# geobacter-rs/rav1e

Hardware: AMD Instinct MI355X
Metric: encoded frames/sec + Mpixels/sec, 4K 8-bit speed=10, 1/2/4/8 GPU vs host CPU (higher is better)
Workload: dtype u8

## Files before the change

rav1e_amd/csrc/rv_rdo.h:

```cpp
#pragma once

#include "rv_chain.h"
#include "rv_device.h"
#include "rv_quant.h"

namespace rv {

struct RdoPlane {
  rv_plane org;
  rv_plane ref[2];
  rv_plane dst;
  int32_t *levels;
  uint64_t *out;
  QCtx q;
};

struct RdoWinner {
  int32_t c;
  int32_t skip;
  double cost;
  uint64_t dist;
};

struct RdoArgs {
  RdoPlane p[2];
  CandGeo g;
  const rv_fs_result *sub;
  const RdoWinner *win;
  const float *imp;
  int w_in_b, h_in_b, w_imp;
  int n_tx;
  int cand_base;
  const int32_t *list;
  const int32_t *count;
  int commit;
  int ntx_per_cand;
  int bd;
  int bsize;
  int mb_w, mb_h;
  int sub_w, sub_h;
  int xdec, ydec;
  int q_tx_index;
  int tx_size, qindex;
  const void *iedges;
  const uint8_t *imodes;
  const uint8_t *iwin;
};

}

int rv_quant_ctx(int qindex, int tx_area, int is_intra, int bit_depth, int dc_delta_q,
                 int ac_delta_q, rv::QCtx *out);

int rv_rdo_candidates(const rv::RdoArgs &luma, const rv::RdoArgs &chroma, int hbd,
                      hipStream_t s, bool compound = false);

int rv_rdo_blocks2(const rv::RdoArgs &l, const rv::RdoArgs &c, int nl, int nc, int hbd,
                   hipStream_t s, int mode);
int rv_rdo_blocks(const rv::RdoArgs &a, bool luma, int nplanes, int n_tx_size, int hbd,
                  hipStream_t s, int mode);

int rv_rdo_args_put(const rv::RdoArgs *h, int n, rv::RdoArgs *dev, hipStream_t s);
int rv_rdo_candidates_list(const rv::RdoArgs *h, const rv::RdoArgs *dev, int nsets, int mode_a,
                           int hbd, hipStream_t s, int max_grid = 0, uint32_t *kp_cnt = nullptr,
                           unsigned long long *kp_t = nullptr);

int rv_rdo_intra(const rv::RdoArgs &luma, const rv::RdoArgs &chroma, int hbd, hipStream_t s);
```

rav1e_amd/csrc/rv_rdo.hip:

```cpp
#include <stdio.h>
#include <stdlib.h>
#include <string.h>

#include <type_traits>

#include "rv_intra.h"
#include "rv_rdo.h"
#include "rv_tx.h"

namespace rv {


__constant__ int8_t kRdoReg[2][16][8] = {
    {{0, 0, 0, 127, 0, 0, 0, 0}, {0, 2, -6, 126, 8, -2, 0, 0},
     {0, 2, -10, 122, 18, -4, 0, 0}, {0, 2, -12, 116, 28, -8, 2, 0},
     {0, 2, -14, 110, 38, -10, 2, 0}, {0, 2, -14, 102, 48, -12, 2, 0},
     {0, 2, -16, 94, 58, -12, 2, 0}, {0, 2, -14, 84, 66, -12, 2, 0},
     {0, 2, -14, 76, 76, -14, 2, 0}, {0, 2, -12, 66, 84, -14, 2, 0},
     {0, 2, -12, 58, 94, -16, 2, 0}, {0, 2, -12, 48, 102, -14, 2, 0},
     {0, 2, -10, 38, 110, -14, 2, 0}, {0, 2, -8, 28, 116, -12, 2, 0},
     {0, 0, -4, 18, 122, -10, 2, 0}, {0, 0, -2, 8, 126, -6, 2, 0}},
    {{0, 0, 0, 127, 0, 0, 0, 0}, {0, 0, -4, 126, 8, -2, 0, 0},
     {0, 0, -8, 122, 18, -4, 0, 0}, {0, 0, -10, 116, 28, -6, 0, 0},
     {0, 0, -12, 110, 38, -8, 0, 0}, {0, 0, -12, 102, 48, -10, 0, 0},
// ... 81 lines not shown
  wave_sync();
  IntraSetup st = intra_setup(jb.imode, jb.ivar);
  if (st.mode == 0) st.dcv = intra_dc<G>(e, jb.ivar, N, N, bd, lane);
  const int maxv = (1 << bd) - 1;
  for (int i = lane; i < N * N; i += G) {
    const int r = i / N, c = i - r * N;
    pred[i] = (Px)intra_px(st, e, N, N, r, c, maxv);
  }
  wave_sync();
}

__device__ __forceinline__ int rdo_ntx(const RdoArgs &a) {
  return a.count ? __builtin_amdgcn_readfirstlane(*a.count) * a.ntx_per_cand : a.n_tx;
}

template <int N>
__device__ __forceinline__ RdoJob rdo_job(const RdoArgs &a, const RdoPlane &pl, int t) {
  const int ci = t / a.ntx_per_cand, sub = t - ci * a.ntx_per_cand;
  const int cand = a.list ? a.list[ci] : a.cand_base + ci;
  int sb, c;
  RdoJob j;
  j.zero = false;
  j.oi = cand * a.ntx_per_cand + sub;
  if (a.commit) {
    sb = cand;
    c = a.win[sb].c;
    j.zero = a.win[sb].skip != 0;
  } else {
    c = cand / a.g.nsb;
    sb = cand - c * a.g.nsb;
  }
  rv_mv mv, mv1{0, 0};
  j.comp = c >= a.g.R * a.g.M;
  if (j.comp) {
// ... 11 lines not shown
  j.oy = (sub / txc) * N;
  const rv_mc_job m = mc_job_for(pl.ref[j.ref], j.bx, j.by, mv, 0, 0);
  j.src_x = m.src_x;
  j.src_y = m.src_y;
  j.cf = m.col_frac;
  j.rf = m.row_frac;
  j.src2_x = j.src2_y = j.cf2 = j.rf2 = 0;
  if (j.comp) {
    const rv_mc_job m1 = mc_job_for(pl.ref[1], j.bx, j.by, mv1, 0, 0);
    j.src2_x = m1.src_x;
    j.src2_y = m1.src_y;
    j.cf2 = m1.col_frac;
    j.rf2 = m1.row_frac;
  }
  return j;
}

struct McF {
  uint32_t xp[3];
  int xsum;
  int yt[8];
  int cf, rf;
};
template <typename Px>
__device__ __forceinline__ McF mc_setup(int cf, int rf, int w, int h) {
  McF f;
  f.cf = cf;
  f.rf = rf;
  const int8_t *xf = kRdoReg[w <= 4][cf];
  const int8_t *yf = kRdoReg[h <= 4][rf];
// ... 220 lines not shown
  }
}

template <typename Px, int N>
__host__ __device__ constexpr int rdo_slab_bytes() {
  constexpr int B = (int)sizeof(Px);
  constexpr int P = B == 1 ? ((N + 8 + 15) / 16) * 16 : ((2 * (N + 8) + 15) / 16) * 16;
  constexpr int RB = N < 16 ? N : 16;
  constexpr int a = N * (N + 1) * 4, b = (N + 7) * P, c = 2 * (RB + 7) * P;
  return ((a > b ? a : b) > c ? (a > b ? a : b) : c);
}

template <typename Px, int N, int LPB, int MODE, bool LUMA = false>
__device__ __forceinline__ void rdo_cand_body(const RdoArgs &a, const RdoPlane &pl, int t,
                                              bool valid, int32_t *buf, Px *pred,
                                              const uint16_t *scan) {
  constexpr int B = (int)sizeof(Px);
  constexpr int S = N + 1;
  constexpr int G = LPB / N, RG = N / G;
  constexpr int U = RG < 8 ? RG : 8;
  constexpr int P = B == 1 ? ((N + 8 + 15) / 16) * 16 : ((2 * (N + 8) + 15) / 16) * 16;
  constexpr int C32 = N < 32 ? N : 32;
  static_assert(!LUMA || N >= 8, "cdef distortion runs on 8x8 blocks");
  const int lane = rv_tid() & (LPB - 1);
  RdoJob jb;
  if constexpr (MODE == 3)
    jb = rdo_job_intra<Px, N>(a, &pl == &a.p[1] ? 2 : 1, t);
  else
    jb = rdo_job<N>(a, pl, t);
  const rv_plane &ref = pl.ref[jb.ref];
  const int ox = jb.ox, oy = jb.oy;
  const int bd = a.bd, ib = bd == 12 ? 2 : 4, maxv = (1 << bd) - 1;
  const int sx0 = jb.bx + ox, sy0 = jb.by + oy;
  auto wave_sync = [] {
    __builtin_amdgcn_fence(__ATOMIC_RELEASE, "wavefront");
    __builtin_amdgcn_wave_barrier();
    __builtin_amdgcn_fence(__ATOMIC_ACQUIRE, "wavefront");
  };

  if constexpr (MODE == 3) {
    intra_fill<Px, N, LPB>(jb, buf, pred, a.bd, lane);
  } else if (MODE == 1 || (MODE == 2 && jb.comp)) {
    static_assert(2 * (16 + 7) * (sizeof(Px) == 1 ? 48 : 80) <= N * (N + 1) * 4 || N != 32,
                  "compound windows must fit the coefficient slab");
// ... 205 lines not shown
#pragma unroll 8
    for (int i = lane; i < N * DPR; i += LPB) {
      const int r = i / DPR, c = (i - r * DPR) * PPD;
      uint32_t v;
      __builtin_memcpy(&v, pred + r * N + c, 4);
      if (valid) __builtin_memcpy(dp + r * ds + c * B, &v, 4);
    }
    return;
  }
  const uint64_t d = group_sum<LPB>(rdo_dist_biased<Px, N, LPB, LUMA>(a, jb, o, ost, pred));
  if (valid && lane == 0) pl.out[(int64_t)jb.oi * 3 + 1] = d;
}

__host__ __device__ constexpr int cmax(int a, int b) { return a > b ? a : b; }

template <typename Px, typename Mid, int NPART>
struct LumaLds {
  static constexpr int kWinP = sizeof(Px) == 1 ? 80 : 144;
  static constexpr int kWinRows = 64 / NPART + 7;
  static constexpr int kCompRows = sizeof(Px) == 1 ? 16 : 8;
  static constexpr int kScr =
      cmax(cmax(cmax(kWinRows * kWinP, 16 * 65 * 4), 32 * 66 * (int)sizeof(Mid)),
           2 * (kCompRows + 7) * kWinP);
  static constexpr int kSlot = (kScr + 64 * 64 * (int)sizeof(Px) + 15) / 16 * 16;
};


template <typename Px>
__device__ __forceinline__ uint64_t luma_dist(const RdoArgs &a, const RdoJob &j, const Px *o,
                                              int64_t os, const Px *pred) {
  const int lane = rv_tid() & 63, by = lane >> 3, bx = lane & 7;
  const uint64_t v =
      rdo_cdef_8x8<Px>(o + (int64_t)(by * 8) * os + bx * 8, os, pred + by * 8 * 64 + bx * 8, 64, a.bd);
  const int px = j.bx + bx * 8, py = j.by + by * 8;
  return group_sum<64>(rdo_biased(v, rdo_bias(a, px >> 2, py >> 2)));
}

template <typename Px, int NPART, int MODE>
__device__ __forceinline__ void luma_front(const RdoArgs &a, const RdoPlane &pl, int t,
                                           const RdoJob &jb, bool valid, uint8_t *scr, Px *pred,
                                           bool skip_dist = true) {
  constexpr int N = 64, B = (int)sizeof(Px);
  constexpr int P = LumaLds<Px, int16_t, NPART>::kWinP;
  constexpr int RP = N / NPART;
  static_assert(RP % 8 == 0, "MC rows run in groups of 8");
  const int lane = rv_tid() & 63;
  const rv_plane &ref = pl.ref[jb.ref];
  const int ox = 0, oy = 0;
  const int bd = a.bd, ib = bd == 12 ? 2 : 4, maxv = (1 << bd) - 1;

  if constexpr (MODE == 3) {
    intra_fill<Px, 64, 64>(jb, reinterpret_cast<int32_t *>(scr), pred, bd, lane);
  } else if (MODE == 1 || (MODE == 2 && jb.comp)) {
    mc_compound<Px, 64, LumaLds<Px, int16_t, NPART>::kCompRows>(
        a, pl, jb, reinterpret_cast<uint32_t *>(scr), pred);
  } else
  {
    uint32_t *win = reinterpret_cast<uint32_t *>(scr);
    const int cf = jb.cf, rf = jb.rf;
    const int8_t *xf = kRdoReg[a.mb_w <= 4][cf];
    const int8_t *yf = kRdoReg[a.mb_h <= 4][rf];
    int yt[8];
#pragma unroll
    for (int k = 0; k < 8; k++) yt[k] = yf[k];
    uint32_t xp[4];
// ... 72 lines not shown
          if (rf) {
            int32_t s = 0;
#pragma unroll
            for (int k = 1; k < 7; k++) s += __mul24(yt[k], ring[(u + k) & 7]);
            v = round_shift(s, vshift);
          } else {
            v = cf ? round_shift(ring[(u + 3) & 7], ib) : ring[(u + 3) & 7];
          }
          pred[(RP * half + r) * N + col] = (Px)clamp_med3(v, 0, maxv);
        }
      }
    }
    wave_sync();
  }

  const Px *o = plane_ptr<Px>(pl.org, jb.bx, jb.by);
  if (!a.commit && skip_dist) {
    const uint64_t d = luma_dist<Px>(a, jb, o, pl.org.stride, pred);
    if (valid && lane == 0) pl.out[(int64_t)jb.oi * 3 + 0] = d;
  }
  int s0, s1, s2;
  fwd_shifts<N>((bd - 8) / 2, s0, s1, s2);
  int32_t *fmid = reinterpret_cast<int32_t *>(scr);
  {
    int32_t v[N];
#pragma unroll
    for (int r = 0; r < N; r++) {
      const int16_t d = (int16_t)((int16_t)o[(int64_t)r * pl.org.stride + lane] -
                                  (int16_t)pred[r * N + lane]);
      v[r] = rdo_rsa((int32_t)d, -s0);
// ... 167 lines not shown
  if (b < luma.n_tx && b >= rdo_ntx(luma)) return;
  if (b < luma.n_tx)
    rdo_luma_body<Px, Mid, 2, MODE>(luma, luma.p[0], b, lds,
                              reinterpret_cast<Px *>(lds + L::kScr), scan);
  else
    rdo_chroma_pair<Px, MODE>(chroma, b - luma.n_tx, reinterpret_cast<int32_t *>(lds),
                        reinterpret_cast<Px *>(lds + 2 * 32 * 33 * 4), scan);
}

template <typename Px>
struct QuadLds {
  using L = LumaLds<Px, int16_t, sizeof(Px) == 1 ? 2 : 4>;
  static constexpr int kBytes = cmax(4 * L::kSlot, 3 * kChromaPair(sizeof(Px)));
};

#ifndef RV_RDO_PHASES
#define RV_RDO_PHASES 0
#endif
__device__ unsigned long long g_rdo_ph[3][8];
struct QuadPh {
  unsigned long long t[5];
};

template <typename Px, int MODE>
__device__ __forceinline__ void rdo_quad_luma(const RdoArgs &luma, int b, int n, int var,
                                              uint8_t *lds, const uint16_t *scan,
                                              QuadPh *ph = nullptr) {
  using L = typename QuadLds<Px>::L;
  constexpr int NPART = sizeof(Px) == 1 ? 2 : 4;
  const int wave = __builtin_amdgcn_readfirstlane(rv_tid() >> 6), lane = rv_tid() & 63;
  auto slot = [&](int q) __attribute__((always_inline)) { return lds + q * L::kSlot; };
  auto fmid = [&](int q) __attribute__((always_inline)) {
    return reinterpret_cast<int32_t *>(slot(q));
  };
  auto imid = [&](int q) __attribute__((always_inline)) {
    return reinterpret_cast<int16_t *>(slot(q));
  };
  auto pred = [&](int q) __attribute__((always_inline)) {
    return reinterpret_cast<Px *>(slot(q) + L::kScr);
  };
  const int t0 = 4 * b, t = t0 + wave;
  if (t0 >= n) return;
  const bool valid = t < n;
  RdoJob jb;
  if constexpr (MODE == 3)
    jb = rdo_job_intra<Px, 64>(luma, 0, valid ? t : n - 1);
  else
    jb = rdo_job<64>(luma, luma.p[0], valid ? t : n - 1);
  const bool late_dist = (var & 1) && !luma.commit;
  const bool prio = (var & 2) != 0;
  if (valid)
    luma_front<Px, NPART, MODE>(luma, luma.p[0], t, jb, true, slot(wave), pred(wave), !late_dist);
  __syncthreads();
  if (RV_RDO_PHASES && ph) ph->t[1] = wall_clock64();
  if (wave == 0) {
    if (prio) __builtin_amdgcn_s_setprio(2);
    const int q = lane >> 4;
    if (t0 + q < n) luma_fwd_row(fmid(q) + (lane & 15) * 65, luma.bd);
    if (prio) __builtin_amdgcn_s_setprio(0);
  } else if (late_dist && valid) {
    const uint64_t d = luma_dist<Px>(luma, jb, plane_ptr<Px>(luma.p[0].org, jb.bx, jb.by),
                                     luma.p[0].org.stride, pred(wave));
    if (lane == 0) luma.p[0].out[(int64_t)jb.oi * 3 + 0] = d;
  }
  __syncthreads();
  if (RV_RDO_PHASES && ph) ph->t[2] = wall_clock64();
  if (valid) luma_quantize(luma, luma.p[0], t, jb, true, fmid(wave), scan);
// ... 2 lines not shown
  if (wave < 2) {
    if (prio) __builtin_amdgcn_s_setprio(2);
    const int q = 2 * wave + (lane >> 5), rr = lane & 31;
    const bool vq = t0 + q < n;
    const int range = luma.bd + 8, crange = luma.bd + 6 > 16 ? luma.bd + 6 : 16;
    int32_t v[64];
    if (vq) luma_inv_row_load(fmid(q), rr, v, range, nullptr);
    wave_sync();
    if (vq) luma_inv_row_tx(v, imid(q) + rr * 66, range, crange);
    if (prio) __builtin_amdgcn_s_setprio(0);
  } else if (wave == 2 && late_dist) {
    RdoJob j0;
    if constexpr (MODE == 3)
      j0 = rdo_job_intra<Px, 64>(luma, 0, t0);
    else
      j0 = rdo_job<64>(luma, luma.p[0], t0);
    const uint64_t d = luma_dist<Px>(luma, j0, plane_ptr<Px>(luma.p[0].org, j0.bx, j0.by),
                                     luma.p[0].org.stride, pred(0));
    if (lane == 0) luma.p[0].out[(int64_t)j0.oi * 3 + 0] = d;
  }
  __syncthreads();
  if (RV_RDO_PHASES && ph) ph->t[4] = wall_clock64();
  if (valid) luma_back<Px, int16_t>(luma, luma.p[0], t, jb, true, imid(wave), pred(wave));
}

template <typename Px, int MODE>
__device__ __forceinline__ void rdo_quad_chroma(const RdoArgs &chroma, int c, int pairs,
                                                uint8_t *lds, const uint16_t *scan) {
  const int wave = __builtin_amdgcn_readfirstlane(rv_tid() >> 6);
  const int pair = 3 * c + wave;
  if (wave == 3 || pair >= 2 * pairs) return;
  uint8_t *w = lds + wave * kChromaPair(sizeof(Px));
  rdo_chroma_pair<Px, MODE>(chroma, pair, reinterpret_cast<int32_t *>(w),
                            reinterpret_cast<Px *>(w + 2 * 32 * 33 * 4), scan, pairs);
}

template <typename Px, int MODE>
__device__ __forceinline__ void rdo_quad_chroma4(const RdoArgs &chroma, int c, int n, uint8_t *lds,
                                                 const uint16_t *scan) {
  constexpr int kSlab = rdo_slab_bytes<Px, 32>();
  static_assert(4 * (kSlab + 32 * 32 * (int)sizeof(Px)) <= QuadLds<Px>::kBytes, "4 chroma slabs");
  const int wave = __builtin_amdgcn_readfirstlane(rv_tid() >> 6);
  const int k = 4 * c + wave;
  if (k >= 2 * n) return;
  const int plane = k >= n ? 1 : 0, i = k - plane * n;
  uint8_t *w = lds + wave * (kSlab + 32 * 32 * (int)sizeof(Px));
  rdo_cand_body<Px, 32, 64, MODE>(chroma, chroma.p[plane], i, true, reinterpret_cast<int32_t *>(w),
                                  reinterpret_cast<Px *>(w + kSlab), scan);
}

template <typename Px, int MODE>
__device__ __forceinline__ void rdo_quad_wg(RdoArgs luma, RdoArgs chroma, int nquads,
                                            int var, int b, uint8_t *lds, uint16_t *scan) {
  if (b >= nquads) {
    const int pairs = (chroma.n_tx + 1) / 2, nc = rdo_ntx(chroma);
    bool any = false;
    for (int w = 0; w < 3; w++) {
      const int p = 3 * (b - nquads) + w;
      if (p < 2 * pairs) any |= 2 * (p - (p / pairs) * pairs) < nc;
    }
    if (!any) return;
  } else if (4 * b >= rdo_ntx(luma)) {
    return;
// ... 1 lines not shown
  stage_scan(scan, b >= nquads ? chroma.q_tx_index : luma.q_tx_index);
  if (b >= nquads)
    rdo_quad_chroma<Px, MODE>(chroma, b - nquads, (chroma.n_tx + 1) / 2, lds, scan);
  else
    rdo_quad_luma<Px, MODE>(luma, b, rdo_ntx(luma), var, lds, scan);
}

template <typename Px, int MODE>
__global__ __launch_bounds__(256) __attribute__((amdgpu_waves_per_eu(4))) void rdo_quad_kernel(
    RdoArgs luma, RdoArgs chroma, int nquads, int var) {
  __shared__ __align__(16) uint8_t lds[QuadLds<Px>::kBytes];
  __shared__ uint16_t scan[1024];
  rdo_quad_wg<Px, MODE>(luma, chroma, nquads, var, blockIdx.x, lds, scan);
}

template <typename Px, int MA, int MB>
__global__ __launch_bounds__(256) __attribute__((amdgpu_waves_per_eu(4))) void rdo_quad_list_kernel(
    const RdoArgs *__restrict__ A, int nsets, int var, uint32_t *kp_cnt, unsigned long long *kp_t) {
  __shared__ __align__(16) uint8_t lds[QuadLds<Px>::kBytes];
  __shared__ uint16_t scan[1024];
  if (kp_t && threadIdx.x == 0) atomicMin(kp_t, (unsigned long long)wall_clock64());
  const RdoArgs &la = A[0], &ca = A[1], &lb = A[2], &cb = A[3];
  const int na = rdo_ntx(la), ma = rdo_ntx(ca);
  const int nb = nsets > 1 ? rdo_ntx(lb) : 0, mb = nsets > 1 ? rdo_ntx(cb) : 0;
  if (kp_cnt && blockIdx.x == 0 && threadIdx.x == 0) {
    atomicAdd(kp_cnt + (MA ? 1 : 0), (uint32_t)na);
    atomicAdd(kp_cnt + (MA ? 3 : 2), (uint32_t)ma);
    if (nsets > 1) {
      atomicAdd(kp_cnt + (MB ? 1 : 0), (uint32_t)nb);
      atomicAdd(kp_cnt + (MB ? 3 : 2), (uint32_t)mb);
    }
  }
  const int pa = (ma + 1) / 2, pb = (mb + 1) / 2;
  const bool c4 = (var & 32) != 0;
  const int e0 = (na + 3) / 4, e1 = e0 + (c4 ? (2 * ma + 3) / 4 : (2 * pa + 2) / 3);
  const int e2 = e1 + (nb + 3) / 4, e3 = e2 + (c4 ? (2 * mb + 3) / 4 : (2 * pb + 2) / 3);
  const bool phd = RV_RDO_PHASES && (var & 16) && rv_tid() == 0;
  for (int b = blockIdx.x; b < e3; b += gridDim.x) {
    QuadPh ph;
    ph.t[0] = phd ? wall_clock64() : 0;
    QuadPh *pp = phd ? &ph : nullptr;
    int set = 2;
    if (b < e0) {
      stage_scan(scan, la.q_tx_index);
      rdo_quad_luma<Px, MA>(la, b, na, var, lds, scan, pp);
      set = MA;
    } else if (b < e1) {
      stage_scan(scan, ca.q_tx_index);
      if (c4)
        rdo_quad_chroma4<Px, MA>(ca, b - e0, ma, lds, scan);
      else
        rdo_quad_chroma<Px, MA>(ca, b - e0, pa, lds, scan);
    } else if (b < e2) {
      stage_scan(scan, lb.q_tx_index);
      rdo_quad_luma<Px, MB>(lb, b - e1, nb, var, lds, scan, pp);
      set = MB;
    } else {
      stage_scan(scan, cb.q_tx_index);
      if (c4)
        rdo_quad_chroma4<Px, MB>(cb, b - e2, mb, lds, scan);
      else
        rdo_quad_chroma<Px, MB>(cb, b - e2, pb, lds, scan);
    }
    __syncthreads();
    if (phd) {
      const unsigned long long te = wall_clock64();
      if (set < 2) {
        for (int k = 0; k < 4; k++) atomicAdd(&g_rdo_ph[set][k], ph.t[k + 1] - ph.t[k]);
        atomicAdd(&g_rdo_ph[set][4], te - ph.t[4]);
      } else {
        atomicAdd(&g_rdo_ph[2][0], te - ph.t[0]);
      }
      atomicAdd(&g_rdo_ph[set][5], 1ull);
    }
  }
  if (kp_t && threadIdx.x == 0) atomicMax(kp_t + 1, (unsigned long long)wall_clock64());
}

__global__ __launch_bounds__(256) void rdo_args_store_kernel(RdoArgs a0, RdoArgs a1, RdoArgs a2,
                                                              RdoArgs a3, int n, RdoArgs *out) {
  static_assert(sizeof(RdoArgs) % 4 == 0, "word copy");
  constexpr int W = (int)(sizeof(RdoArgs) / 4);
  for (int i = threadIdx.x; i < n * W; i += blockDim.x) {
    const int k = i / W, w = i - k * W;
// ... 146 lines not shown
      h[0].commit || h[0].bd == 12)
    return rv_set_error(RV_EINVAL, "rv_rdo_candidates_list: bad arguments");
  for (int k = 0; k < 2 * nsets; k++)
    if (!h[k].list || !h[k].count)
      return rv_set_error(RV_EINVAL, "rv_rdo_candidates_list: the sets must be list-driven");
  static const bool phases = getenv("RAV1E_HIP_RDO_PHASES") && getenv("RAV1E_HIP_RDO_PHASES")[0] == '1';
  const int var = kRdoVariant | (phases && max_grid > 0 ? 16 : 0) | (max_grid > 0 ? 32 : 0);
  unsigned full = 0;
  for (int k = 0; k < nsets; k++)
    full += (unsigned)((h[2 * k].n_tx + 3) / 4) +
            ((var & 32) ? (unsigned)(2 * h[2 * k + 1].n_tx + 3) / 4
                        : (unsigned)(2 * ((h[2 * k + 1].n_tx + 1) / 2) + 2) / 3);
  unsigned grid = std::min(full, kF4Pool);
  if (max_grid > 0) grid = std::min(grid, (unsigned)max_grid);
  if (grid == 0) return RV_OK;
#define RV_LIST(PX, MA, MB) \
  rdo_quad_list_kernel<PX, MA, MB><<<grid, 256, 0, s>>>(dev, nsets, var, kp_cnt, kp_t)
  if (hbd) {
    if (nsets == 2) RV_LIST(uint16_t, 0, 1); else if (mode_a) RV_LIST(uint16_t, 1, 1); else RV_LIST(uint16_t, 0, 0);
  } else {
    if (nsets == 2) RV_LIST(uint8_t, 0, 1); else if (mode_a) RV_LIST(uint8_t, 1, 1); else RV_LIST(uint8_t, 0, 0);
  }
#undef RV_LIST
  RV_HIP_CHECK_LAUNCH();
  return RV_OK;
}

int rv_rdo_intra(const RdoArgs &luma, const RdoArgs &chroma, int hbd, hipStream_t s) {
  const unsigned cpairs = (unsigned)(2 * ((chroma.n_tx + 1) / 2));
  rdo_launch<3>(luma, chroma, hbd, s, cpairs);
  RV_HIP_CHECK_LAUNCH();
  return RV_OK;
}

int rv_rdo_blocks2(const RdoArgs &l, const RdoArgs &c, int nl, int nc, int hbd, hipStream_t s,
                   int mode) {
  if (nl == 32 && nc == 16) rdo_small2_launch<32, 16>(l, c, hbd, s, mode);
  else if (nl == 16 && nc == 8) rdo_small2_launch<16, 8>(l, c, hbd, s, mode);
// ... 21 lines not shown
    else return rv_set_error(RV_EINVAL, "rv_rdo_blocks: chroma size");
  }
  RV_HIP_CHECK_LAUNCH();
  return RV_OK;
}

extern "C" int rv_rdo_phase_dump(void) {
  unsigned long long h[3][8];
  if (hipDeviceSynchronize() != hipSuccess || hipMemcpyFromSymbol(h, HIP_SYMBOL(g_rdo_ph), sizeof(h)) != hipSuccess)
    return rv_set_error(RV_EHIP, "rv_rdo_phase_dump");
  const double us = 0.01;
  static const char *kName[2] = {"single", "compound"};
  for (int m = 0; m < 2; m++) {
    const double n = h[m][5] ? (double)h[m][5] : 1.0;
    fprintf(stderr,
            "[f4 phases] %s luma quads %llu: front %.2f, row DCT %.2f, quantize %.2f, inverse rows %.2f, "
            "back %.2f us per quad\n",
            kName[m], h[m][5], h[m][0] * us / n, h[m][1] * us / n, h[m][2] * us / n, h[m][3] * us / n,
            h[m][4] * us / n);
  }
  fprintf(stderr, "[f4 phases] chroma triples %llu: %.2f us each\n", h[2][5],
          h[2][0] * us / (h[2][5] ? (double)h[2][5] : 1.0));
  memset(h, 0, sizeof(h));
  return hipMemcpyToSymbol(HIP_SYMBOL(g_rdo_ph), h, sizeof(h)) == hipSuccess ? RV_OK
                                                                           : rv_set_error(RV_EHIP, "rv_rdo_phase_dump");
}
```

rav1e_amd/csrc/rv_replay.hip:

```cpp
#include <string.h>

#include <chrono>
#include <condition_variable>
#include <algorithm>
#include <deque>
#include <mutex>
#include <thread>
#include <vector>

#include "rv_chain.h"
#include "rv_device.h"
#include "rv_ec.h"
#include "rv_intra.h"
#include "rv_intra_pass.h"
#include "rv_mvref.h"
#include "rv_impwin.h"
#include "rv_lrf.h"
#include "rv_rdo.h"
#include <string>

#if __has_include(<rccl/rccl.h>)
#include <rccl/rccl.h>
#define RV_HAVE_RCCL 1
#else
// ... 168 lines not shown
                                         const uint64_t *lout, const uint64_t *uout,
                                         const uint64_t *vout, int ntx_c, int sb) {
  RdoWinner w{0, 0, 1.7976931348623157e308, 0};
  for (int c = 0; c < cg.R * cg.M + cg.comp; c++)
    argmin_step(w, cand_cost(cg, lambda, ds_u, ds_v, sub, lout, uout, vout, ntx_c, sb, c), c);
  return w;
}

constexpr int kScoreMaxCands = 2 * kCandModes + kCompModes;
__global__ __launch_bounds__(256) void score_wave_kernel(
    Geo g, CandGeo cg, double lambda, double ds_u, double ds_v, const rv_fs_result *sub,
    const uint64_t *lout, const uint64_t *uout, const uint64_t *vout, int ntx_c, RdoWinner *win,
    const rv_fs_result *coarse, const rv_fs_result *half, const rv_fs_result *full,
    const rv_fs_result *look, const rv_fs_result *half_l, uint64_t *words, int32_t *cand_count,
    unsigned long long *imp_sum, uint32_t *evals, int32_t *leaf_count, const int32_t *alist,
    const int32_t *acount, BlkDec *dec, int round) {
  __shared__ CandCost kc[4][kScoreMaxCands];
  __shared__ RdoWinner ws[4];
  const int wave = threadIdx.x >> 6, lane = threadIdx.x & 63;
  const int n = alist ? __builtin_amdgcn_readfirstlane(*acount) : g.nsb;
  const int nc = cg.R * cg.M + cg.comp;
  const int per = kWordsPerRef * g.R + 4;
  for (int i = blockIdx.x * 4 + wave; i < n; i += gridDim.x * 4) {
    const int sb = alist ? __builtin_amdgcn_readfirstlane(alist[i]) : i;
    if (lane < nc)
      kc[wave][lane] = cand_cost(cg, lambda, ds_u, ds_v, sub, lout, uout, vout, ntx_c, sb, lane);
    wave_sync();
    if (lane == 0) {
      RdoWinner w{0, 0, 1.7976931348623157e308, 0};
      for (int c = 0; c < nc; c++) argmin_step(w, kc[wave][c], c);
      ws[wave] = w;
      win[sb] = w;
      if (dec) dec[sb] = blk_dec_of(cg, sub, sb, w.c);
    }
    wave_sync();
    const RdoWinner w = ws[wave];
    uint64_t *base = words + (int64_t)sb * per;
    for (int wi = lane; wi < per; wi += 64) {
      uint64_t v;
      if (wi < kWordsPerRef * g.R) {
        const int r = wi / kWordsPerRef, k = wi - r * kWordsPerRef, e = k >> 1;
// ... 128 lines not shown
  const int lane = threadIdx.x & 63;
  const uint64_t below = (1ull << lane) - 1;
  const uint64_t bh = __ballot(mh), bl = __ballot(ml);
  int b0 = 0, b1 = 0;
  if (lane == 0) {
    if (bh) b0 = atomicAdd(a.pub.cnt, (int)__popcll(bh));
    if (bl) b1 = atomicAdd(a.pub.cnt + 1, (int)__popcll(bl));
  }
  b0 = __shfl(b0, 0, 64);
  b1 = __shfl(b1, 0, 64);
  if (mh) a.list_h[b0 + __popcll(bh & below)] = job;
  if (ml) a.list_l[b1 + __popcll(bl & below)] = job;
  round_publish(a.pub);
}

struct CandKey {
  uint32_t tag, mv0, mv1;
};
struct CandKeys {
  CandKey *key;
  uint32_t tag;
  int reuse;
};
__device__ inline uint32_t mv_bits(rv_mv m) {
  return (uint32_t)(uint16_t)m.row | ((uint32_t)(uint16_t)m.col << 16);
}
__device__ inline bool cand_key_step(const CandKeys &k, int slot, bool v, rv_mv m0, rv_mv m1) {
  if (!v || !k.key) return v;
  const CandKey n{k.tag, mv_bits(m0), mv_bits(m1)};
  const CandKey o = k.key[slot];
  if (k.reuse && o.tag == n.tag && o.mv0 == n.mv0 && o.mv1 == n.mv1) return false;
  k.key[slot] = n;
  return true;
}

__global__ __launch_bounds__(256) void cand_list_kernel(CandGeo cg, const rv_fs_result *sub,
                                                         int n, int32_t *list, int32_t *count,
                                                         const uint8_t *active = nullptr,
                                                         CandKeys keys = CandKeys{nullptr, 0, 0}) {
  const int i = blockIdx.x * 256 + threadIdx.x;
  bool v = false;
// ... 2818 lines not shown
    ma.count = slot_cnt(q);
    ma.pub = r->rr.pub(q);
    ma.list = mvl(q);
    RV_R(rv_mvref_round(ma, st));
  }
  if (r->exact) {
    RV_R(rv_diamond_search_multi(&cur.hres, refs_h, g.R, r->jobs_half[lv], nr * 4, 16, 16, 0, 0, 0,
                                 g.bd, r->half, nullptr, nullptr, st));
  } else {
    RV_H(hipMemcpyAsync(r->half, r->half_l, (size_t)nr * g.R * 4 * sizeof(rv_fs_result),
                        hipMemcpyDeviceToDevice, st));
    fill_preds_kernel<<<(nr * g.R + 255) / 256, 256, 0, st>>>(r->jobs_full[lv], r->src_full,
                                                              nr * g.R, r->coarse, r->half, 0);
  }
  const uint8_t *act = r->exact ? r->mv_active : nullptr;
  const RdoArgs la4 = la, ca4 = ca;
  RdoArgs lc4 = la4, cc4 = ca4;
  lc4.list = cc4.list = r->cand_list + nsingle;
  lc4.count = cc4.count = r->cand_count + 1;
  lc4.cand_base = cc4.cand_base = 0;
  lc4.n_tx = g.nsb * cg.comp;
  cc4.n_tx = g.nsb * cg.comp * ntx_c;
  const RdoArgs f4h[4] = {la4, ca4, lc4, cc4};
  const bool f4_list = g.bd != 12;
  if (f4_list) RV_R(rv_rdo_args_put(f4h, cg.comp ? 4 : 2, r->f4_args, st));
  auto f3_f4 = [&]() -> int {
    RV_R(rv_diamond_search_multi(&cur.y, refs_y, g.R, r->jobs_full[lv], nr, 64, 64, 0, 0, 0, g.bd,
                                 r->full, ev_full, &to_sub, st, act));
    RV_EV(5);
    RV_R(kp_open(st));
    RV_R(rv_diamond_search_multi(&cur.y, refs_y, g.R, r->jobs_sub[lv], nr, 64, 64, 1,
// ... 44 lines not shown
    int lg = q == q_first ? nr * g.R : 0;
    const int hint = q == q_first ? -1 : r->rr.last_count;
    const int hsb = hint >= 0 ? std::max(2 * hint, 16) : 0;
    int f4_grid = 0;
    if (hsb) {
      lg = std::min(hsb * g.R, 512);
      f4_grid = std::min(6 * hsb, 1024);
    }
    RV_R(kp_open(xs));
    RV_R(rv_diamond_f2_f3(&cur.hres, refs_h, r->jobs_half[lv], r->half, ma.f2dirty, &cur.y,
                          refs_y, r->jobs_full[lv], r->full, ma.f3dirty, &to_sub, g.R, nr, g.bd,
                          mvl(q), acnt, lg, xs, r->jobs_sub[lv], r->sub, kp_acc, kp_ts()));
    RV_R(kp_close(xs));
    const int rg = hsb ? std::min(kRoundGrid, std::max((14 * hsb + 255) / 256, (hsb + 3) / 4))
                       : kRoundGrid;
    round_lists_kernel<<<rg, 256, 0, xs>>>(
        cg, r->sub, nsingle, r->cand_list, r->cand_count, mvl(q), acnt,
        CandKeys{r->cand_key, (uint32_t)(r->coded + 1), 1});
    if (f4_list) {
      RV_R(kp_open(xs, 1));
      RV_R(rv_rdo_candidates_list(f4h, r->f4_args, cg.comp ? 2 : 1, 0, g.hbd, xs, f4_grid, kp_f4,
                                  kp_ts(1)));
      RV_R(kp_close(xs, 1));
    } else {
      RV_R(rv_rdo_candidates(la4, ca4, g.hbd, xs));
      if (cg.comp) RV_R(rv_rdo_candidates(lc4, cc4, g.hbd, xs, true));
    }
    score_wave_kernel<<<rg, 256, 0, xs>>>(
        g, cg, L.lambda, L.ds[1], L.ds[2], r->sub, r->l_out, r->c_out, r->c_out + nct * 3, ntx_c,
        r->win, r->coarse, r->half, r->full, r->look, r->half_l, r->words, r->cand_count, nullptr,
        nullptr, nullptr, mvl(q), acnt, r->dec_lv[lv], 1);
    return RV_OK;
  };
  RV_R(f3_f4());
  const int budget = g.tws + 2 * g.ths - 2;
  int mv_runs = 0;
  auto mv_rounds_run = [&](const uint8_t *iwas, bool *changed) -> int {
    mv_runs++;
    q_first = r->rr.seq;
    return rounds(
        st, budget,
        [&](uint32_t q) {
          ma.init = 0;
          ma.iwas = iwas;
          ma.count = slot_cnt(q);
          ma.pub = r->rr.pub(q);
// ... 522 lines not shown
```

Measured before the change: 182.0.

## Enumerate RDO candidates per superblock in-kernel, skipping round_lists pass

In later MV refinement rounds, the RDO list kernel gains a per-superblock mode. Each wave recomputes candidate liveness itself and checks it against cached MV keys with a ballot mask, so the separate round_lists_kernel launch and global candidate lists are no longer needed. The score kernel now writes the candidate keys after scoring, so unchanged candidates are skipped in the next round. This removes a launch and a list compaction step, at the cost of a grid sized per superblock that may contain many idle blocks, plus extra key traffic. Phase timing instrumentation for MC and setup is also added.

New measurement: 176.7. 2.9% lower.

```diff
diff --git a/rav1e_amd/csrc/rv_rdo.h b/rav1e_amd/csrc/rv_rdo.h
--- a/rav1e_amd/csrc/rv_rdo.h
+++ b/rav1e_amd/csrc/rv_rdo.h
@@ -22,6 +22,18 @@
   uint64_t dist;
 };
 
+struct CandKey {
+  uint32_t tag, mv0, mv1;
+};
+struct CandKeys {
+  CandKey *key;
+  uint32_t tag;
+  int reuse;
+};
+__host__ __device__ inline uint32_t mv_bits(rv_mv m) {
+  return (uint32_t)(uint16_t)m.row | ((uint32_t)(uint16_t)m.col << 16);
+}
+
 struct RdoArgs {
   RdoPlane p[2];
   CandGeo g;
@@ -45,6 +57,8 @@
   const void *iedges;
   const uint8_t *imodes;
   const uint8_t *iwin;
+  const CandKey *keys;
+  uint32_t key_tag;
 };
 
 }
@@ -64,5 +78,9 @@
 int rv_rdo_candidates_list(const rv::RdoArgs *h, const rv::RdoArgs *dev, int nsets, int mode_a,
                            int hbd, hipStream_t s, int max_grid = 0, uint32_t *kp_cnt = nullptr,
                            unsigned long long *kp_t = nullptr);
+int rv_rdo_sb_slots(int nsingle_modes, int comp_modes, int ntx_per_cand);
+int rv_rdo_candidates_sb(const rv::RdoArgs *h, const rv::RdoArgs *dev, int nsets, int hbd,
+                         hipStream_t s, const int32_t *sbl, const int32_t *sbn, int hsb,
+                         uint32_t *kp_cnt = nullptr, unsigned long long *kp_t = nullptr);
 
 int rv_rdo_intra(const rv::RdoArgs &luma, const rv::RdoArgs &chroma, int hbd, hipStream_t s);
diff --git a/rav1e_amd/csrc/rv_rdo.hip b/rav1e_amd/csrc/rv_rdo.hip
--- a/rav1e_amd/csrc/rv_rdo.hip
+++ b/rav1e_amd/csrc/rv_rdo.hip
@@ -119,10 +119,19 @@
   return a.count ? __builtin_amdgcn_readfirstlane(*a.count) * a.ntx_per_cand : a.n_tx;
 }
 
+struct SbPick {
+  uint32_t mask;
+  int base;
+  __device__ __forceinline__ int cand(int k, int nsb) const {
+    uint32_t m = mask;
+    for (int i = 0; i < k; i++) m &= m - 1;
+    return base + __builtin_ctz(m) * nsb;
+  }
+};
+
 template <int N>
-__device__ __forceinline__ RdoJob rdo_job(const RdoArgs &a, const RdoPlane &pl, int t) {
-  const int ci = t / a.ntx_per_cand, sub = t - ci * a.ntx_per_cand;
-  const int cand = a.list ? a.list[ci] : a.cand_base + ci;
+__device__ __forceinline__ RdoJob rdo_job_cand(const RdoArgs &a, const RdoPlane &pl, int cand,
+                                               int sub) {
   int sb, c;
   RdoJob j;
   j.zero = false;
@@ -164,6 +173,13 @@
     j.rf2 = m1.row_frac;
   }
   return j;
+}
+template <int N>
+__device__ __forceinline__ RdoJob rdo_job(const RdoArgs &a, const RdoPlane &pl, int t,
+                                          SbPick pk = SbPick{0, 0}) {
+  const int ci = t / a.ntx_per_cand, sub = t - ci * a.ntx_per_cand;
+  const int cand = pk.mask ? pk.cand(ci, a.g.nsb) : a.list ? a.list[ci] : a.cand_base + ci;
+  return rdo_job_cand<N>(a, pl, cand, sub);
 }
 
 struct McF {
@@ -414,7 +430,7 @@
 template <typename Px, int N, int LPB, int MODE, bool LUMA = false>
 __device__ __forceinline__ void rdo_cand_body(const RdoArgs &a, const RdoPlane &pl, int t,
                                               bool valid, int32_t *buf, Px *pred,
-                                              const uint16_t *scan) {
+                                              const uint16_t *scan, SbPick pk = SbPick{0, 0}) {
   constexpr int B = (int)sizeof(Px);
   constexpr int S = N + 1;
   constexpr int G = LPB / N, RG = N / G;
@@ -427,7 +443,7 @@
   if constexpr (MODE == 3)
     jb = rdo_job_intra<Px, N>(a, &pl == &a.p[1] ? 2 : 1, t);
   else
-    jb = rdo_job<N>(a, pl, t);
+    jb = rdo_job<N>(a, pl, t, pk);
   const rv_plane &ref = pl.ref[jb.ref];
   const int ox = jb.ox, oy = jb.oy;
   const int bd = a.bd, ib = bd == 12 ? 2 : 4, maxv = (1 << bd) - 1;
@@ -663,6 +679,13 @@
 
 __host__ __device__ constexpr int cmax(int a, int b) { return a > b ? a : b; }
 
+struct QuadPh {
+  unsigned long long t[5], m[2];
+};
+#ifndef RV_RDO_PHASES
+#define RV_RDO_PHASES 0
+#endif
+
 template <typename Px, typename Mid, int NPART>
 struct LumaLds {
   static constexpr int kWinP = sizeof(Px) == 1 ? 80 : 144;
@@ -688,7 +711,7 @@
 template <typename Px, int NPART, int MODE>
 __device__ __forceinline__ void luma_front(const RdoArgs &a, const RdoPlane &pl, int t,
                                            const RdoJob &jb, bool valid, uint8_t *scr, Px *pred,
-                                           bool skip_dist = true) {
+                                           bool skip_dist = true, QuadPh *ph = nullptr) {
   constexpr int N = 64, B = (int)sizeof(Px);
   constexpr int P = LumaLds<Px, int16_t, NPART>::kWinP;
   constexpr int RP = N / NPART;
@@ -698,6 +721,7 @@
   const int ox = 0, oy = 0;
   const int bd = a.bd, ib = bd == 12 ? 2 : 4, maxv = (1 << bd) - 1;
 
+  if (RV_RDO_PHASES && ph) ph->m[0] = wall_clock64();
   if constexpr (MODE == 3) {
     intra_fill<Px, 64, 64>(jb, reinterpret_cast<int32_t *>(scr), pred, bd, lane);
   } else if (MODE == 1 || (MODE == 2 && jb.comp)) {
@@ -800,6 +824,7 @@
     wave_sync();
   }
 
+  if (RV_RDO_PHASES && ph) ph->m[1] = wall_clock64();
   const Px *o = plane_ptr<Px>(pl.org, jb.bx, jb.by);
   if (!a.commit && skip_dist) {
     const uint64_t d = luma_dist<Px>(a, jb, o, pl.org.stride, pred);
@@ -997,18 +1022,12 @@
   static constexpr int kBytes = cmax(4 * L::kSlot, 3 * kChromaPair(sizeof(Px)));
 };
 
-#ifndef RV_RDO_PHASES
-#define RV_RDO_PHASES 0
-#endif
 __device__ unsigned long long g_rdo_ph[3][8];
-struct QuadPh {
-  unsigned long long t[5];
-};
 
 template <typename Px, int MODE>
 __device__ __forceinline__ void rdo_quad_luma(const RdoArgs &luma, int b, int n, int var,
                                               uint8_t *lds, const uint16_t *scan,
-                                              QuadPh *ph = nullptr) {
+                                              QuadPh *ph = nullptr, SbPick pk = SbPick{0, 0}) {
   using L = typename QuadLds<Px>::L;
   constexpr int NPART = sizeof(Px) == 1 ? 2 : 4;
   const int wave = __builtin_amdgcn_readfirstlane(rv_tid() >> 6), lane = rv_tid() & 63;
@@ -1029,11 +1048,12 @@
   if constexpr (MODE == 3)
     jb = rdo_job_intra<Px, 64>(luma, 0, valid ? t : n - 1);
   else
-    jb = rdo_job<64>(luma, luma.p[0], valid ? t : n - 1);
+    jb = rdo_job<64>(luma, luma.p[0], valid ? t : n - 1, pk);
   const bool late_dist = (var & 1) && !luma.commit;
   const bool prio = (var & 2) != 0;
   if (valid)
-    luma_front<Px, NPART, MODE>(luma, luma.p[0], t, jb, true, slot(wave), pred(wave), !late_dist);
+    luma_front<Px, NPART, MODE>(luma, luma.p[0], t, jb, true, slot(wave), pred(wave), !late_dist,
+                                ph);
   __syncthreads();
   if (RV_RDO_PHASES && ph) ph->t[1] = wall_clock64();
   if (wave == 0) {
@@ -1066,7 +1086,7 @@
     if constexpr (MODE == 3)
       j0 = rdo_job_intra<Px, 64>(luma, 0, t0);
     else
-      j0 = rdo_job<64>(luma, luma.p[0], t0);
+      j0 = rdo_job<64>(luma, luma.p[0], t0, pk);
     const uint64_t d = luma_dist<Px>(luma, j0, plane_ptr<Px>(luma.p[0].org, j0.bx, j0.by),
                                      luma.p[0].org.stride, pred(0));
     if (lane == 0) luma.p[0].out[(int64_t)j0.oi * 3 + 0] = d;
@@ -1089,7 +1109,7 @@
 
 template <typename Px, int MODE>
 __device__ __forceinline__ void rdo_quad_chroma4(const RdoArgs &chroma, int c, int n, uint8_t *lds,
-                                                 const uint16_t *scan) {
+                                                 const uint16_t *scan, SbPick pk = SbPick{0, 0}) {
   constexpr int kSlab = rdo_slab_bytes<Px, 32>();
   static_assert(4 * (kSlab + 32 * 32 * (int)sizeof(Px)) <= QuadLds<Px>::kBytes, "4 chroma slabs");
   const int wave = __builtin_amdgcn_readfirstlane(rv_tid() >> 6);
@@ -1098,7 +1118,7 @@
   const int plane = k >= n ? 1 : 0, i = k - plane * n;
   uint8_t *w = lds + wave * (kSlab + 32 * 32 * (int)sizeof(Px));
   rdo_cand_body<Px, 32, 64, MODE>(chroma, chroma.p[plane], i, true, reinterpret_cast<int32_t *>(w),
-                                  reinterpret_cast<Px *>(w + kSlab), scan);
+                                  reinterpret_cast<Px *>(w + kSlab), scan, pk);
 }
 
 template <typename Px, int MODE>
@@ -1130,16 +1150,22 @@
   rdo_quad_wg<Px, MODE>(luma, chroma, nquads, var, blockIdx.x, lds, scan);
 }
 
+__host__ __device__ constexpr int rdo_sb_slots(int ns, int comp, int ntc) {
+  return (ns + 3) / 4 + (2 * ns * ntc + 3) / 4 + (comp + 3) / 4 + (2 * comp * ntc + 3) / 4;
+}
+
 template <typename Px, int MA, int MB>
 __global__ __launch_bounds__(256) __attribute__((amdgpu_waves_per_eu(4))) void rdo_quad_list_kernel(
-    const RdoArgs *__restrict__ A, int nsets, int var, uint32_t *kp_cnt, unsigned long long *kp_t) {
+    const RdoArgs *__restrict__ A, int nsets, int var, uint32_t *kp_cnt, unsigned long long *kp_t,
+    const int32_t *__restrict__ sbl, const int32_t *__restrict__ sbn) {
   __shared__ __align__(16) uint8_t lds[QuadLds<Px>::kBytes];
   __shared__ uint16_t scan[1024];
   if (kp_t && threadIdx.x == 0) atomicMin(kp_t, (unsigned long long)wall_clock64());
   const RdoArgs &la = A[0], &ca = A[1], &lb = A[2], &cb = A[3];
-  const int na = rdo_ntx(la), ma = rdo_ntx(ca);
-  const int nb = nsets > 1 ? rdo_ntx(lb) : 0, mb = nsets > 1 ? rdo_ntx(cb) : 0;
-  if (kp_cnt && blockIdx.x == 0 && threadIdx.x == 0) {
+  const bool sbm = (var & 64) != 0;
+  const int na = sbm ? 0 : rdo_ntx(la), ma = sbm ? 0 : rdo_ntx(ca);
+  const int nb = nsets > 1 && !sbm ? rdo_ntx(lb) : 0, mb = nsets > 1 && !sbm ? rdo_ntx(cb) : 0;
+  if (kp_cnt && !sbm && blockIdx.x == 0 && threadIdx.x == 0) {
     atomicAdd(kp_cnt + (MA ? 1 : 0), (uint32_t)na);
     atomicAdd(kp_cnt + (MA ? 3 : 2), (uint32_t)ma);
     if (nsets > 1) {
@@ -1149,34 +1175,78 @@
   }
   const int pa = (ma + 1) / 2, pb = (mb + 1) / 2;
   const bool c4 = (var & 32) != 0;
-  const int e0 = (na + 3) / 4, e1 = e0 + (c4 ? (2 * ma + 3) / 4 : (2 * pa + 2) / 3);
-  const int e2 = e1 + (nb + 3) / 4, e3 = e2 + (c4 ? (2 * mb + 3) / 4 : (2 * pb + 2) / 3);
+  int e0, e1, e2, e3, items;
+  if (sbm) {
+    const int ns = la.g.R * la.g.M, nc = la.g.comp, ntc = ca.ntx_per_cand;
+    e0 = (ns + 3) / 4, e1 = e0 + (2 * ns * ntc + 3) / 4;
+    e2 = e1 + (nc + 3) / 4, e3 = e2 + (2 * nc * ntc + 3) / 4;
+    items = __builtin_amdgcn_readfirstlane(*sbn) * e3;
+  } else {
+    e0 = (na + 3) / 4, e1 = e0 + (c4 ? (2 * ma + 3) / 4 : (2 * pa + 2) / 3);
+    e2 = e1 + (nb + 3) / 4, e3 = e2 + (c4 ? (2 * mb + 3) / 4 : (2 * pb + 2) / 3);
+    items = e3;
+  }
   const bool phd = RV_RDO_PHASES && (var & 16) && rv_tid() == 0;
-  for (int b = blockIdx.x; b < e3; b += gridDim.x) {
+  for (int b = blockIdx.x; b < items; b += gridDim.x) {
+    const int ent = sbm ? __builtin_amdgcn_readfirstlane(b / e3) : 0, s = b - ent * e3;
+    const int kind = s < e0 ? 0 : s < e1 ? 1 : s < e2 ? 2 : 3;
+    const int idx = s - (kind == 0 ? 0 : kind == 1 ? e0 : kind == 2 ? e1 : e2);
+    int n;
+    SbPick pk{0, 0};
+    if (sbm) {
+      const RdoArgs *L = A;
+      const CandGeo &cg = L[0].g;
+      const int sb = __builtin_amdgcn_readfirstlane(sbl[ent]);
+      const int ns = cg.R * cg.M, lane = rv_tid() & 63;
+      const int c = (kind < 2 ? 0 : ns) + lane;
+      bool v = false;
+      if (lane < (kind < 2 ? ns : cg.comp)) {
+        rv_mv m0, m1{0, 0};
+        if (kind < 2) {
+          v = cand_live(cg, L[0].sub, sb, c, &m0);
+        } else {
+          v = comp_live(cg, L[0].sub, sb, lane);
+          if (v) comp_mvs(cg, L[0].sub, sb, lane, &m0, &m1);
+        }
+        if (v) {
+          const CandKey o = L[0].keys[c * cg.nsb + sb];
+          v = !(o.tag == L[0].key_tag && o.mv0 == mv_bits(m0) && o.mv1 == mv_bits(m1));
+        }
+      }
+      pk = SbPick{(uint32_t)__ballot(v), (kind < 2 ? 0 : ns) * cg.nsb + sb};
+      n = __popc(pk.mask) * ((kind & 1) ? L[1].ntx_per_cand : 1);
+      if (4 * idx >= ((kind & 1) ? 2 * n : n)) continue;
+      if (kp_cnt && rv_tid() == 0) {
+        const int u = (n < 4 * idx + 4 ? n : 4 * idx + 4) - 4 * idx;
+        if (u > 0) atomicAdd(kp_cnt + ((kind < 2 ? MA : MB) ? 1 : 0) + ((kind & 1) ? 2 : 0), (uint32_t)u);
+      }
+    } else {
+      n = kind == 0 ? na : kind == 1 ? ma : kind == 2 ? nb : mb;
+    }
     QuadPh ph;
     ph.t[0] = phd ? wall_clock64() : 0;
     QuadPh *pp = phd ? &ph : nullptr;
     int set = 2;
-    if (b < e0) {
+    if (kind == 0) {
       stage_scan(scan, la.q_tx_index);
-      rdo_quad_luma<Px, MA>(la, b, na, var, lds, scan, pp);
+      rdo_quad_luma<Px, MA>(la, idx, n, var, lds, scan, pp, pk);
       set = MA;
-    } else if (b < e1) {
+    } else if (kind == 1) {
       stage_scan(scan, ca.q_tx_index);
       if (c4)
-        rdo_quad_chroma4<Px, MA>(ca, b - e0, ma, lds, scan);
+        rdo_quad_chroma4<Px, MA>(ca, idx, n, lds, scan, pk);
       else
-        rdo_quad_chroma<Px, MA>(ca, b - e0, pa, lds, scan);
-    } else if (b < e2) {
+        rdo_quad_chroma<Px, MA>(ca, idx, pa, lds, scan);
+    } else if (kind == 2) {
       stage_scan(scan, lb.q_tx_index);
-      rdo_quad_luma<Px, MB>(lb, b - e1, nb, var, lds, scan, pp);
+      rdo_quad_luma<Px, MB>(lb, idx, n, var, lds, scan, pp, pk);
       set = MB;
     } else {
       stage_scan(scan, cb.q_tx_index);
       if (c4)
-        rdo_quad_chroma4<Px, MB>(cb, b - e2, mb, lds, scan);
+        rdo_quad_chroma4<Px, MB>(cb, idx, n, lds, scan, pk);
       else
-        rdo_quad_chroma<Px, MB>(cb, b - e2, pb, lds, scan);
+        rdo_quad_chroma<Px, MB>(cb, idx, pb, lds, scan);
     }
     __syncthreads();
     if (phd) {
@@ -1184,6 +1254,8 @@
       if (set < 2) {
         for (int k = 0; k < 4; k++) atomicAdd(&g_rdo_ph[set][k], ph.t[k + 1] - ph.t[k]);
         atomicAdd(&g_rdo_ph[set][4], te - ph.t[4]);
+        atomicAdd(&g_rdo_ph[set][6], ph.m[1] - ph.m[0]);
+        atomicAdd(&g_rdo_ph[set][7], ph.t[1] - ph.m[1]);
       } else {
         atomicAdd(&g_rdo_ph[2][0], te - ph.t[0]);
       }
@@ -1360,14 +1432,43 @@
   unsigned grid = std::min(full, kF4Pool);
   if (max_grid > 0) grid = std::min(grid, (unsigned)max_grid);
   if (grid == 0) return RV_OK;
-#define RV_LIST(PX, MA, MB) \
-  rdo_quad_list_kernel<PX, MA, MB><<<grid, 256, 0, s>>>(dev, nsets, var, kp_cnt, kp_t)
+#define RV_LIST(PX, MA, MB)                                                                  \
+  rdo_quad_list_kernel<PX, MA, MB><<<grid, 256, 0, s>>>(dev, nsets, var, kp_cnt, kp_t, nullptr, \
+                                                        nullptr)
   if (hbd) {
     if (nsets == 2) RV_LIST(uint16_t, 0, 1); else if (mode_a) RV_LIST(uint16_t, 1, 1); else RV_LIST(uint16_t, 0, 0);
   } else {
     if (nsets == 2) RV_LIST(uint8_t, 0, 1); else if (mode_a) RV_LIST(uint8_t, 1, 1); else RV_LIST(uint8_t, 0, 0);
   }
 #undef RV_LIST
+  RV_HIP_CHECK_LAUNCH();
+  return RV_OK;
+}
+
+int rv_rdo_sb_slots(int nsingle_modes, int comp_modes, int ntx_per_cand) {
+  return rdo_sb_slots(nsingle_modes, comp_modes, ntx_per_cand);
+}
+
+int rv_rdo_candidates_sb(const RdoArgs *h, const RdoArgs *dev, int nsets, int hbd, hipStream_t s,
+                         const int32_t *sbl, const int32_t *sbn, int hsb, uint32_t *kp_cnt,
+                         unsigned long long *kp_t) {
+  if (!h || !dev || nsets < 1 || nsets > 2 || h[0].commit || h[0].bd == 12 || !sbl || !sbn ||
+      !h[0].keys || (nsets == 2) != (h[0].g.comp != 0) || h[0].g.R * h[0].g.M > 32 ||
+      h[0].g.comp > 32)
+    return rv_set_error(RV_EINVAL, "rv_rdo_candidates_sb: bad arguments");
+  static const bool phases = getenv("RAV1E_HIP_RDO_PHASES") && getenv("RAV1E_HIP_RDO_PHASES")[0] == '1';
+  const int var = kRdoVariant | (phases ? 16 : 0) | 32 | 64;
+  const int Q = rdo_sb_slots(h[0].g.R * h[0].g.M, h[0].g.comp, h[1].ntx_per_cand);
+  const unsigned grid = (unsigned)std::min<long>((long)(hsb > 0 ? hsb : h[0].g.nsb) * Q, (long)kF4Pool);
+  if (grid == 0) return RV_OK;
+#define RV_SB(PX, MA, MB) \
+  rdo_quad_list_kernel<PX, MA, MB><<<grid, 256, 0, s>>>(dev, nsets, var, kp_cnt, kp_t, sbl, sbn)
+  if (hbd) {
+    if (nsets == 2) RV_SB(uint16_t, 0, 1); else RV_SB(uint16_t, 0, 0);
+  } else {
+    if (nsets == 2) RV_SB(uint8_t, 0, 1); else RV_SB(uint8_t, 0, 0);
+  }
+#undef RV_SB
   RV_HIP_CHECK_LAUNCH();
   return RV_OK;
 }
@@ -1419,9 +1520,10 @@
   for (int m = 0; m < 2; m++) {
     const double n = h[m][5] ? (double)h[m][5] : 1.0;
     fprintf(stderr,
-            "[f4 phases] %s luma quads %llu: front %.2f, row DCT %.2f, quantize %.2f, inverse rows %.2f, "
-            "back %.2f us per quad\n",
-            kName[m], h[m][5], h[m][0] * us / n, h[m][1] * us / n, h[m][2] * us / n, h[m][3] * us / n,
+            "[f4 phases] %s luma quads %llu: front %.2f (setup + scan %.2f, MC %.2f, residual + column "
+            "DCT %.2f), row DCT %.2f, quantize %.2f, inverse rows %.2f, back %.2f us per quad\n",
+            kName[m], h[m][5], h[m][0] * us / n, (h[m][0] - h[m][6] - h[m][7]) * us / n,
+            h[m][6] * us / n, h[m][7] * us / n, h[m][1] * us / n, h[m][2] * us / n, h[m][3] * us / n,
             h[m][4] * us / n);
   }
   fprintf(stderr, "[f4 phases] chroma triples %llu: %.2f us each\n", h[2][5],
diff --git a/rav1e_amd/csrc/rv_replay.hip b/rav1e_amd/csrc/rv_replay.hip
--- a/rav1e_amd/csrc/rv_replay.hip
+++ b/rav1e_amd/csrc/rv_replay.hip
@@ -206,7 +206,7 @@
     const rv_fs_result *coarse, const rv_fs_result *half, const rv_fs_result *full,
     const rv_fs_result *look, const rv_fs_result *half_l, uint64_t *words, int32_t *cand_count,
     unsigned long long *imp_sum, uint32_t *evals, int32_t *leaf_count, const int32_t *alist,
-    const int32_t *acount, BlkDec *dec, int round) {
+    const int32_t *acount, BlkDec *dec, int round, CandKeys keys = CandKeys{nullptr, 0, 0}) {
   __shared__ CandCost kc[4][kScoreMaxCands];
   __shared__ RdoWinner ws[4];
   const int wave = threadIdx.x >> 6, lane = threadIdx.x & 63;
@@ -215,8 +215,17 @@
   const int per = kWordsPerRef * g.R + 4;
   for (int i = blockIdx.x * 4 + wave; i < n; i += gridDim.x * 4) {
     const int sb = alist ? __builtin_amdgcn_readfirstlane(alist[i]) : i;
-    if (lane < nc)
+    if (lane < nc) {
       kc[wave][lane] = cand_cost(cg, lambda, ds_u, ds_v, sub, lout, uout, vout, ntx_c, sb, lane);
+      if (keys.key && kc[wave][lane].live) {
+        rv_mv m0, m1{0, 0};
+        if (lane < cg.R * cg.M)
+          (void)cand_mv(cg, sub, sb, lane, &m0);
+        else
+          comp_mvs(cg, sub, sb, lane - cg.R * cg.M, &m0, &m1);
+        keys.key[lane * cg.nsb + sb] = CandKey{keys.tag, mv_bits(m0), mv_bits(m1)};
+      }
+    }
     wave_sync();
     if (lane == 0) {
       RdoWinner w{0, 0, 1.7976931348623157e308, 0};
@@ -375,17 +384,6 @@
   round_publish(a.pub);
 }
 
-struct CandKey {
-  uint32_t tag, mv0, mv1;
-};
-struct CandKeys {
-  CandKey *key;
-  uint32_t tag;
-  int reuse;
-};
-__device__ inline uint32_t mv_bits(rv_mv m) {
-  return (uint32_t)(uint16_t)m.row | ((uint32_t)(uint16_t)m.col << 16);
-}
 __device__ inline bool cand_key_step(const CandKeys &k, int slot, bool v, rv_mv m0, rv_mv m1) {
   if (!v || !k.key) return v;
   const CandKey n{k.tag, mv_bits(m0), mv_bits(m1)};
@@ -3234,7 +3232,10 @@
                                                               nr * g.R, r->coarse, r->half, 0);
   }
   const uint8_t *act = r->exact ? r->mv_active : nullptr;
-  const RdoArgs la4 = la, ca4 = ca;
+  RdoArgs la4 = la;
+  la4.keys = r->cand_key;
+  la4.key_tag = (uint32_t)(r->coded + 1);
+  const RdoArgs ca4 = ca;
   RdoArgs lc4 = la4, cc4 = ca4;
   lc4.list = cc4.list = r->cand_list + nsingle;
   lc4.count = cc4.count = r->cand_count + 1;
@@ -3309,10 +3310,17 @@
     RV_R(kp_close(xs));
     const int rg = hsb ? std::min(kRoundGrid, std::max((14 * hsb + 255) / 256, (hsb + 3) / 4))
                        : kRoundGrid;
-    round_lists_kernel<<<rg, 256, 0, xs>>>(
-        cg, r->sub, nsingle, r->cand_list, r->cand_count, mvl(q), acnt,
-        CandKeys{r->cand_key, (uint32_t)(r->coded + 1), 1});
-    if (f4_list) {
+    const CandKeys keys{r->cand_key, (uint32_t)(r->coded + 1), 1};
+    const bool f4_sb = f4_list && q != q_first && ntx_c == 1;
+    if (!f4_sb)
+      round_lists_kernel<<<rg, 256, 0, xs>>>(cg, r->sub, nsingle, r->cand_list, r->cand_count,
+                                             mvl(q), acnt, keys);
+    if (f4_sb) {
+      RV_R(kp_open(xs, 1));
+      RV_R(rv_rdo_candidates_sb(f4h, r->f4_args, cg.comp ? 2 : 1, g.hbd, xs, mvl(q), acnt, hsb, kp_f4,
+                                kp_ts(1)));
+      RV_R(kp_close(xs, 1));
+    } else if (f4_list) {
       RV_R(kp_open(xs, 1));
       RV_R(rv_rdo_candidates_list(f4h, r->f4_args, cg.comp ? 2 : 1, 0, g.hbd, xs, f4_grid, kp_f4,
                                   kp_ts(1)));
@@ -3324,7 +3332,7 @@
     score_wave_kernel<<<rg, 256, 0, xs>>>(
         g, cg, L.lambda, L.ds[1], L.ds[2], r->sub, r->l_out, r->c_out, r->c_out + nct * 3, ntx_c,
         r->win, r->coarse, r->half, r->full, r->look, r->half_l, r->words, r->cand_count, nullptr,
-        nullptr, nullptr, mvl(q), acnt, r->dec_lv[lv], 1);
+        nullptr, nullptr, mvl(q), acnt, r->dec_lv[lv], 1, f4_sb ? keys : CandKeys{nullptr, 0, 0});
     return RV_OK;
   };
   RV_R(f3_f4());
```
